# ai-dynamo/grove

Hardware: AMD Instinct MI355X
Metric: podgangs_per_sec (higher is better)
Workload: dtype bf16; 1 GPU; global_batch=4, parallelism=gang1, gang_size=1, payload=2048x2048x2048x1, inflight=2, concurrent_syncs=4, transport=http, scheduler=amd-gang-scheduler (native xGMI Filter/Score)

## Files before the change

grove_amd/kubelet/gpunode.py:

```python
from __future__ import annotations

import logging
from typing import Any, Dict, Optional, Tuple

from ..api import constants as c
from ..kubecore.store import Obj

log = logging.getLogger("grove.gpunode")

PAYLOAD_ANNOTATION = "grove.io/payload"
PAYLOAD_SHAPE_ANNOTATION = "grove.io/payload-shape"
GPU_IDS_ANNOTATION = "scheduling.amd.com/gpu-ids"

_gpuwork = None


def load_gpuwork():
    global _gpuwork
    if _gpuwork is not None:
        return _gpuwork
    import torch
    try:
        from ..ops import _gpuwork as ext
    except ImportError as e:
        if torch.cuda.is_available():
            raise RuntimeError(
                "grove_amd.ops._gpuwork native extension is missing on a GPU box — "
                "build it with python -m grove_amd.ops.build") from e
        return None
    _gpuwork = ext
    return ext


def parse_payload(pod: Obj) -> Tuple[str, Tuple[int, ...]]:
    ann = pod["metadata"].get("annotations") or {}
    kind = ann.get(PAYLOAD_ANNOTATION, "gemm")
    shape = ann.get(PAYLOAD_SHAPE_ANNOTATION, "")
    if kind == "gemm":
        dims = tuple(int(x) for x in shape.split("x")) if shape else (1024, 1024, 1024, 1)
        if len(dims) == 3:
            dims = dims + (1,)
        return "gemm", dims
    if kind == "stream":
        return "stream", (int(shape) if shape else 1 << 24, 2)
    if kind == "decode":
        dims = tuple(int(v) for v in shape.split("x")) if shape else (8192, 8192, 4)
        if len(dims) == 2:
            dims = dims + (1,)
        return "decode", dims
    return "none", ()


def assigned_gpu(pod: Obj) -> Optional[int]:
    ids = (pod["metadata"].get("annotations") or {}).get(GPU_IDS_ANNOTATION, "")
    if not ids:
        return None
    return int(ids.split(",")[0])


def run_payload_descriptor(kind: str, dims: Tuple[int, ...], device: int) -> Dict[str, Any]:
    import torch
    if not torch.cuda.is_available():
        if kind == "gemm":
            m, n, k, iters = dims
            a = torch.randn(min(m, 128), min(k, 128))
            b = torch.randn(min(k, 128), min(n, 128))
            for _ in range(iters):
                a @ b
        return {"device": "cpu", "kind": kind}
    ext = load_gpuwork()
    device = device % max(1, torch.cuda.device_count())
    with torch.cuda.device(device):
        if kind == "gemm":
            m, n, k, iters = dims
            tflops = ext.burn_gemm(m, n, k, iters)
            return {"device": device, "kind": kind, "tflops": tflops}
        if kind == "stream":
            n_floats = dims[0]
            iters = dims[1] if len(dims) > 1 else 2
            gbps = ext.stream_triad(n_floats, iters)
            return {"device": device, "kind": kind, "gbps": gbps}
        if kind == "decode":
            n, k, iters = dims
            gbps = ext.burn_decode(n, k, iters)
            return {"device": device, "kind": kind, "weight_stream_gbps": gbps}
    return {"device": device, "kind": kind}


def gpu_pod_payload(pod: Obj) -> None:
    gpu = assigned_gpu(pod)
    kind, dims = parse_payload(pod)
    if kind == "none":
        return
    if gpu is None:
        gpu = 0
    run_payload_descriptor(kind, dims, gpu)
```

grove_amd/ops/gpuwork.hip:

```cpp
#include <torch/extension.h>
#include <ATen/hip/HIPContext.h>
#include <hip/hip_runtime.h>
#include <hip/hip_bf16.h>

#include <vector>

#define WAVE 64
#define BK 64

using bf16 = __hip_bfloat16;
using bf16x8 = __attribute__((ext_vector_type(8))) __bf16;
using f32x16 = __attribute__((ext_vector_type(16))) float;

__device__ __forceinline__ int swz(int row, int cb) {
    return (cb ^ ((row ^ (row >> 3)) & 7)) & 7;
}

__device__ __forceinline__ int lds_off(int row, int cb) {
    return row * BK + (swz(row, cb) << 3);
}

__device__ __forceinline__ void tile_map(int bid, int num_pid_m, int tiles_n,
                                         int& tile_m, int& tile_n) {
    const int GROUP = 8;
    int group_size = min(GROUP, num_pid_m);
    int pids_per_group = group_size * tiles_n;
    int group = bid / pids_per_group;
    int in_group = bid % pids_per_group;
    tile_m = group * GROUP + (in_group % group_size);
    tile_n = in_group / group_size;
}

__device__ __forceinline__ void tile_map_rect(int bid, int tiles_m, int tiles_n,
                                              int m_per_xcd, int n_win,
                                              int& tile_m, int& tile_n) {
    int mwin_tiles = 8 * m_per_xcd;
    int win = bid >> 8;
    int idx = bid & 255;
    int xcd = idx & 7;
    int slot = idx >> 3;
    int nwins = tiles_n / n_win;
    tile_m = (win / nwins) * mwin_tiles + xcd * m_per_xcd + slot % m_per_xcd;
    tile_n = (win % nwins) * n_win + slot / m_per_xcd;
}

template <int THREADS, int AUX = 0>
__device__ __forceinline__ void stage_tile(const bf16* __restrict__ g, long ld,
                                           __bf16* __restrict__ dst, int rows,
                                           int tid, int wave_piece0) {
#pragma unroll
    for (int i = 0; i < 8; ++i) {
        if (i >= (rows * 8) / THREADS)
            break;
        int p = tid + i * THREADS;
        int row = p >> 3;
        int cb_src = swz(row, p & 7);
        int base = wave_piece0 + i * THREADS;
        __builtin_amdgcn_global_load_lds(
            (const __attribute__((address_space(1))) uint32_t*)(
                g + (long)row * ld + (cb_src << 3)),
            (__attribute__((address_space(3))) uint32_t*)(dst + base * 8),
            16, 0, AUX);
    }
}

__global__ __launch_bounds__(512, 1)
void mfma_gemm_bf16_256_kernel(const bf16* __restrict__ A,
                               const bf16* __restrict__ Bt,
                               float* __restrict__ C,
                               int M, int N, int K,
                               int m_per_xcd, int n_win) {
    constexpr int BM = 256, BN = 256;
    __shared__ __bf16 smem[2 * (BM * BK + BN * BK)];
    auto sAp = [&](int b) { return smem + b * (BM * BK + BN * BK); };
    auto sBp = [&](int b) { return smem + b * (BM * BK + BN * BK) + BM * BK; };

    int tile_m, tile_n;
    if (m_per_xcd)
        tile_map_rect(blockIdx.x, M / BM, N / BN, m_per_xcd, n_win,
                      tile_m, tile_n);
    else
        tile_map(blockIdx.x, M / BM, N / BN, tile_m, tile_n);
    const int tid = threadIdx.x;
    const int wave = tid / WAVE;
    const int lane = tid % WAVE;
    const int wr = wave >> 1, wc = wave & 1;
    const long row0 = (long)tile_m * BM;
    const long col0 = (long)tile_n * BN;
    const int wave_piece0 = wave * WAVE;

    auto stage = [&](int buf, long kk) {
        stage_tile<512>(A + row0 * K + kk, K, sAp(buf), BM, tid, wave_piece0);
        stage_tile<512>(Bt + col0 * K + kk, K, sBp(buf), BN, tid, wave_piece0);
    };

    f32x16 acc[2][4] = {};
    bf16x8 afrag[2][2], bfrag[2][4];
    const int a_row = wr * 64 + (lane & 31);
    const int b_row = wc * 128 + (lane & 31);
    const int k_half = lane >> 5;
    auto load_frags = [&](int pb, int buf, int ks) {
        int cb = (ks << 1) | k_half;
#pragma unroll
        for (int mt = 0; mt < 2; ++mt)
            afrag[pb][mt] = *(const bf16x8*)(sAp(buf) + lds_off(a_row + mt * 32, cb));
#pragma unroll
        for (int nt = 0; nt < 4; ++nt)
            bfrag[pb][nt] = *(const bf16x8*)(sBp(buf) + lds_off(b_row + nt * 32, cb));
    };

    stage(0, 0);
    __syncthreads();
    load_frags(0, 0, 0);
    for (long kk = 0; kk < K; kk += BK) {
        int buf = (kk / BK) & 1;
        if (kk + BK < K) stage(buf ^ 1, kk + BK);
#pragma unroll
        for (int ks = 0; ks < BK / 16; ++ks) {
            int pb = ks & 1;
            if (ks + 1 < BK / 16)
                load_frags(pb ^ 1, buf, ks + 1);
#pragma unroll
            for (int mt = 0; mt < 2; ++mt)
#pragma unroll
                for (int nt = 0; nt < 4; ++nt)
                    acc[mt][nt] = __builtin_amdgcn_mfma_f32_32x32x16_bf16(
                        afrag[pb][mt], bfrag[pb][nt], acc[mt][nt], 0, 0, 0);
        }
        __syncthreads();
        if (kk + BK < K) load_frags(0, buf ^ 1, 0);
    }

    const int c_row_lane = 4 * (lane >> 5);
#pragma unroll
    for (int mt = 0; mt < 2; ++mt)
#pragma unroll
        for (int nt = 0; nt < 4; ++nt)
#pragma unroll
            for (int reg = 0; reg < 16; ++reg) {
                int r = wr * 64 + mt * 32 + (reg & 3) + 8 * (reg >> 2) + c_row_lane;
                int cl = wc * 128 + nt * 32 + (lane & 31);
                C[(row0 + r) * (long)N + col0 + cl] = acc[mt][nt][reg];
            }
}

__global__ __launch_bounds__(256, 2)
void mfma_gemm_bf16_128_kernel(const bf16* __restrict__ A,
                               const bf16* __restrict__ Bt,
                               float* __restrict__ C,
                               int M, int N, int K) {
    constexpr int BM = 128, BN = 128;
    __shared__ __bf16 smem[2 * (BM * BK + BN * BK)];
    auto sAp = [&](int b) { return smem + b * (BM * BK + BN * BK); };
    auto sBp = [&](int b) { return smem + b * (BM * BK + BN * BK) + BM * BK; };

    int tile_m, tile_n;
    tile_map(blockIdx.x, M / BM, N / BN, tile_m, tile_n);
    const int tid = threadIdx.x;
    const int wave = tid / WAVE;
    const int lane = tid % WAVE;
    const int wr = wave >> 1, wc = wave & 1;
    const long row0 = (long)tile_m * BM;
    const long col0 = (long)tile_n * BN;
    const int wave_piece0 = wave * WAVE;

    auto stage = [&](int buf, long kk) {
        stage_tile<256>(A + row0 * K + kk, K, sAp(buf), BM, tid, wave_piece0);
        stage_tile<256>(Bt + col0 * K + kk, K, sBp(buf), BN, tid, wave_piece0);
    };

    f32x16 acc[2][2] = {};
    bf16x8 afrag[2][2], bfrag[2][2];
    const int a_row = wr * 64 + (lane & 31);
    const int b_row = wc * 64 + (lane & 31);
    const int k_half = lane >> 5;
    auto load_frags = [&](int pb, int buf, int ks) {
        int cb = (ks << 1) | k_half;
#pragma unroll
        for (int mt = 0; mt < 2; ++mt)
            afrag[pb][mt] = *(const bf16x8*)(sAp(buf) + lds_off(a_row + mt * 32, cb));
#pragma unroll
        for (int nt = 0; nt < 2; ++nt)
            bfrag[pb][nt] = *(const bf16x8*)(sBp(buf) + lds_off(b_row + nt * 32, cb));
    };

    stage(0, 0);
    __syncthreads();
    load_frags(0, 0, 0);
    for (long kk = 0; kk < K; kk += BK) {
        int buf = (kk / BK) & 1;
        if (kk + BK < K) stage(buf ^ 1, kk + BK);
#pragma unroll
        for (int ks = 0; ks < BK / 16; ++ks) {
            int pb = ks & 1;
            if (ks + 1 < BK / 16)
                load_frags(pb ^ 1, buf, ks + 1);
#pragma unroll
            for (int mt = 0; mt < 2; ++mt)
#pragma unroll
                for (int nt = 0; nt < 2; ++nt)
                    acc[mt][nt] = __builtin_amdgcn_mfma_f32_32x32x16_bf16(
                        afrag[pb][mt], bfrag[pb][nt], acc[mt][nt], 0, 0, 0);
        }
        __syncthreads();
        if (kk + BK < K) load_frags(0, buf ^ 1, 0);
    }

    const int c_row_lane = 4 * (lane >> 5);
#pragma unroll
    for (int mt = 0; mt < 2; ++mt)
#pragma unroll
        for (int nt = 0; nt < 2; ++nt)
#pragma unroll
            for (int reg = 0; reg < 16; ++reg) {
                int r = wr * 64 + mt * 32 + (reg & 3) + 8 * (reg >> 2) + c_row_lane;
                int cl = wc * 64 + nt * 32 + (lane & 31);
                C[(row0 + r) * (long)N + col0 + cl] = acc[mt][nt][reg];
            }
}

__global__ __launch_bounds__(256)
void decode_gemv_kernel(const bf16* __restrict__ W,
                        const bf16* __restrict__ x,
                        float* __restrict__ y, int N, int K) {
    const int lane = threadIdx.x % WAVE;
    const int wave = threadIdx.x / WAVE;
    const int row = blockIdx.x * 4 + wave;
    if (row >= N) return;
    const bf16* w = W + (long)row * K;
    float acc = 0.f;
    for (int k0 = lane * 8; k0 < K; k0 += WAVE * 8) {
        bf16x8 wv = *(const bf16x8*)(w + k0);
        bf16x8 xv = *(const bf16x8*)(x + k0);
#pragma unroll
        for (int i = 0; i < 8; ++i)
            acc += (float)wv[i] * (float)xv[i];
    }
    for (int off = 32; off > 0; off >>= 1)
        acc += __shfl_down(acc, off, 64);
    if (lane == 0) y[row] = acc;
}

torch::Tensor decode_gemv(torch::Tensor w, torch::Tensor x) {
    TORCH_CHECK(w.is_cuda() && x.is_cuda() && w.dtype() == torch::kBFloat16
                && x.dtype() == torch::kBFloat16, "bf16 GPU tensors required");
    TORCH_CHECK(w.is_contiguous() && x.is_contiguous(), "contiguous required");
    int64_t N = w.size(0), K = w.size(1);
    TORCH_CHECK(x.numel() == K && K % 512 == 0, "x must be [K], K%512==0");
    auto y = torch::empty({N}, w.options().dtype(torch::kFloat32));
    hipStream_t stream = at::hip::getCurrentHIPStream();
    hipLaunchKernelGGL(decode_gemv_kernel, dim3((N + 3) / 4), dim3(256), 0, stream,
                       (const bf16*)w.data_ptr(), (const bf16*)x.data_ptr(),
                       y.data_ptr<float>(), (int)N, (int)K);
    return y;
}

double burn_decode(int64_t n, int64_t k, int64_t iters) {
    auto opt = torch::TensorOptions().dtype(torch::kBFloat16).device(torch::kCUDA);
    auto w = torch::randn({n, k}, opt.dtype(torch::kFloat32)).to(torch::kBFloat16);
    auto x = torch::randn({k}, opt.dtype(torch::kFloat32)).to(torch::kBFloat16);
    auto y = torch::empty({n}, opt.dtype(torch::kFloat32));
    hipStream_t stream = at::hip::getCurrentHIPStream();
    auto launch = [&] {
        hipLaunchKernelGGL(decode_gemv_kernel, dim3((n + 3) / 4), dim3(256), 0,
                           stream, (const bf16*)w.data_ptr(),
                           (const bf16*)x.data_ptr(), y.data_ptr<float>(),
                           (int)n, (int)k);
    };
    launch();
    C10_HIP_CHECK(hipStreamSynchronize(stream));
    auto t0 = std::chrono::steady_clock::now();
    for (int64_t i = 0; i < iters; ++i) launch();
    C10_HIP_CHECK(hipStreamSynchronize(stream));
    auto t1 = std::chrono::steady_clock::now();
    double secs = std::chrono::duration<double>(t1 - t0).count();
    return 2.0 * n * k * iters / secs / 1e9;
}

__global__ void stream_triad_kernel(const float4* __restrict__ a,
                                    const float4* __restrict__ b,
                                    float4* __restrict__ c, long n4, float s) {
    long i = (long)blockIdx.x * blockDim.x + threadIdx.x;
    long stride = (long)gridDim.x * blockDim.x;
    for (; i < n4; i += stride) {
        float4 x = a[i], y = b[i];
        c[i] = make_float4(x.x + s * y.x, x.y + s * y.y, x.z + s * y.z, x.w + s * y.w);
    }
}


static void launch_gemm(const torch::Tensor& a, const torch::Tensor& bt,
                        torch::Tensor& c, int64_t M, int64_t N, int64_t K,
                        int64_t map_mode = -1) {
    hipStream_t stream = at::hip::getCurrentHIPStream();
    if (M % 256 == 0 && N % 256 == 0 && (M / 256) * (N / 256) >= 256) {
        int tiles_m = (int)(M / 256), tiles_n = (int)(N / 256);
        int m_per_xcd = 0, n_win = 0;
        int mpx = std::min<int>(4, std::max(1, tiles_m / 8));
        int nw = 256 / (8 * mpx);
        bool want_rect = (map_mode == 1) ||
                         (map_mode < 0 && (int64_t)tiles_m * tiles_n > 256);
        if (want_rect && map_mode != 0 &&
            tiles_m % (8 * mpx) == 0 && tiles_n % nw == 0) {
            m_per_xcd = mpx; n_win = nw;
        }
        dim3 grid((M / 256) * (N / 256)), block(512);
        hipLaunchKernelGGL(mfma_gemm_bf16_256_kernel, grid, block, 0, stream,
                           (const bf16*)a.data_ptr(), (const bf16*)bt.data_ptr(),
                           c.data_ptr<float>(), (int)M, (int)N, (int)K,
                           m_per_xcd, n_win);
    } else {
        dim3 grid((M / 128) * (N / 128)), block(256);
        hipLaunchKernelGGL(mfma_gemm_bf16_128_kernel, grid, block, 0, stream,
                           (const bf16*)a.data_ptr(), (const bf16*)bt.data_ptr(),
                           c.data_ptr<float>(), (int)M, (int)N, (int)K);
    }
}

static void check_dims(int64_t M, int64_t N, int64_t K) {
    TORCH_CHECK(M % 128 == 0 && N % 128 == 0 && K % 64 == 0,
                "mfma_gemm_bf16 requires M%128==0, N%128==0, K%64==0 (got ",
                M, "x", N, "x", K, ")");
}

torch::Tensor mfma_gemm_bf16(torch::Tensor a, torch::Tensor bt) {
    TORCH_CHECK(a.is_cuda() && bt.is_cuda(), "inputs must be on GPU");
    TORCH_CHECK(a.dtype() == torch::kBFloat16 && bt.dtype() == torch::kBFloat16,
                "inputs must be bf16");
    TORCH_CHECK(a.is_contiguous() && bt.is_contiguous(), "inputs must be contiguous");
    int64_t M = a.size(0), K = a.size(1), N = bt.size(0);
    TORCH_CHECK(bt.size(1) == K, "shape mismatch: A[M,K] Bt[N,K]");
    check_dims(M, N, K);
    auto c = torch::empty({M, N}, a.options().dtype(torch::kFloat32));
    launch_gemm(a, bt, c, M, N, K);
    return c;
}

double burn_gemm(int64_t m, int64_t n, int64_t k, int64_t iters,
                 int64_t map_mode) {
    check_dims(m, n, k);
    auto opt = torch::TensorOptions().dtype(torch::kBFloat16).device(torch::kCUDA);
    auto a = torch::randn({m, k}, opt.dtype(torch::kFloat32)).to(torch::kBFloat16);
    auto bt = torch::randn({n, k}, opt.dtype(torch::kFloat32)).to(torch::kBFloat16);
    auto c = torch::empty({m, n}, opt.dtype(torch::kFloat32));
    hipStream_t stream = at::hip::getCurrentHIPStream();
    launch_gemm(a, bt, c, m, n, k, map_mode);
    C10_HIP_CHECK(hipStreamSynchronize(stream));
    auto t0 = std::chrono::steady_clock::now();
    for (int64_t i = 0; i < iters; ++i) launch_gemm(a, bt, c, m, n, k, map_mode);
    C10_HIP_CHECK(hipStreamSynchronize(stream));
    auto t1 = std::chrono::steady_clock::now();
    double secs = std::chrono::duration<double>(t1 - t0).count();
    return 2.0 * m * n * k * iters / secs / 1e12;
}

double stream_triad(int64_t n_floats, int64_t iters) {
    TORCH_CHECK(n_floats % 4 == 0, "n_floats must be a multiple of 4");
    auto opt = torch::TensorOptions().dtype(torch::kFloat32).device(torch::kCUDA);
    auto a = torch::randn({n_floats}, opt);
    auto b = torch::randn({n_floats}, opt);
    auto c = torch::empty({n_floats}, opt);
    long n4 = n_floats / 4;
    hipStream_t stream = at::hip::getCurrentHIPStream();
    int blocks = std::min<long>(8192, (n4 + 255) / 256);
    auto launch = [&] {
        hipLaunchKernelGGL(stream_triad_kernel, dim3(blocks), dim3(256), 0, stream,
                           (const float4*)a.data_ptr(), (const float4*)b.data_ptr(),
                           (float4*)c.data_ptr(), n4, 1.5f);
    };
    launch();
    C10_HIP_CHECK(hipStreamSynchronize(stream));
    auto t0 = std::chrono::steady_clock::now();
    for (int64_t i = 0; i < iters; ++i) launch();
    C10_HIP_CHECK(hipStreamSynchronize(stream));
    auto t1 = std::chrono::steady_clock::now();
    double secs = std::chrono::duration<double>(t1 - t0).count();
    return 12.0 * n_floats * iters / secs / 1e9;
}

PYBIND11_MODULE(TORCH_EXTENSION_NAME, m) {
    m.doc() = "grove_amd MI355X pod-payload kernels (MFMA bf16 GEMM, HBM stream)";
    m.def("mfma_gemm_bf16", &mfma_gemm_bf16, "C[M,N]=A[M,K]@Bt[N,K]^T (bf16 in, fp32 out)");
    m.def("burn_gemm", &burn_gemm, "run iters GEMM steps; returns TFLOP/s",
          pybind11::arg("m"), pybind11::arg("n"), pybind11::arg("k"),
          pybind11::arg("iters"), pybind11::arg("map_mode") = -1);
    m.def("burn_gemm_v",
          [](int64_t m_, int64_t n_, int64_t k_, int64_t it, int64_t) {
              return burn_gemm(m_, n_, k_, it, -1);
          }, "compat alias for burn_gemm (bk arg ignored)");
    m.def("stream_triad", &stream_triad, "HBM triad; returns GB/s");
    m.def("decode_gemv", &decode_gemv, "y[N]=W[N,K]@x[K] (bf16 in, fp32 out)");
    m.def("burn_decode", &burn_decode,
          "iters decode GEMV steps; returns weight-stream GB/s");
}
```

Before: 321.8 gangs/s.

## Streamline pod payload: fused bf16 RNG fill, skip warmup, event timing, GIL release

Replaces the fp32 randn-then-cast input generation with a single custom kernel that writes bf16 normals directly, skips the warmup launch for pod payloads, and times with pooled HIP events instead of a stream sync plus a host clock. It also releases the GIL during the native burn calls and passes the device as an argument instead of using a Python context manager. This is meant to cut per-pod GPU work and host serialisation so concurrent payloads overlap. Dropping the warmup could change the reported TFLOP/s, and the custom RNG produces a different distribution quality than torch.randn.

```diff
diff --git a/grove_amd/kubelet/gpunode.py b/grove_amd/kubelet/gpunode.py
--- a/grove_amd/kubelet/gpunode.py
+++ b/grove_amd/kubelet/gpunode.py
@@ -70,20 +70,19 @@
         return {"device": "cpu", "kind": kind}
     ext = load_gpuwork()
     device = device % max(1, torch.cuda.device_count())
-    with torch.cuda.device(device):
-        if kind == "gemm":
-            m, n, k, iters = dims
-            tflops = ext.burn_gemm(m, n, k, iters)
-            return {"device": device, "kind": kind, "tflops": tflops}
-        if kind == "stream":
-            n_floats = dims[0]
-            iters = dims[1] if len(dims) > 1 else 2
-            gbps = ext.stream_triad(n_floats, iters)
-            return {"device": device, "kind": kind, "gbps": gbps}
-        if kind == "decode":
-            n, k, iters = dims
-            gbps = ext.burn_decode(n, k, iters)
-            return {"device": device, "kind": kind, "weight_stream_gbps": gbps}
+    if kind == "gemm":
+        m, n, k, iters = dims
+        tflops = ext.burn_gemm(m, n, k, iters, warmup=False, device=device)
+        return {"device": device, "kind": kind, "tflops": tflops}
+    if kind == "stream":
+        n_floats = dims[0]
+        iters = dims[1] if len(dims) > 1 else 2
+        gbps = ext.stream_triad(n_floats, iters, device=device)
+        return {"device": device, "kind": kind, "gbps": gbps}
+    if kind == "decode":
+        n, k, iters = dims
+        gbps = ext.burn_decode(n, k, iters, warmup=False, device=device)
+        return {"device": device, "kind": kind, "weight_stream_gbps": gbps}
     return {"device": device, "kind": kind}
 
 
diff --git a/grove_amd/ops/gpuwork.hip b/grove_amd/ops/gpuwork.hip
--- a/grove_amd/ops/gpuwork.hip
+++ b/grove_amd/ops/gpuwork.hip
@@ -3,6 +3,13 @@
 #include <hip/hip_runtime.h>
 #include <hip/hip_bf16.h>
 
+#include <ATen/hip/impl/HIPGuardImplMasqueradingAsCUDA.h>
+
+#include <atomic>
+#include <mutex>
+#include <optional>
+#include <random>
+#include <utility>
 #include <vector>
 
 #define WAVE 64
@@ -255,11 +262,131 @@
     return y;
 }
 
-double burn_decode(int64_t n, int64_t k, int64_t iters) {
-    auto opt = torch::TensorOptions().dtype(torch::kBFloat16).device(torch::kCUDA);
-    auto w = torch::randn({n, k}, opt.dtype(torch::kFloat32)).to(torch::kBFloat16);
-    auto x = torch::randn({k}, opt.dtype(torch::kFloat32)).to(torch::kBFloat16);
-    auto y = torch::empty({n}, opt.dtype(torch::kFloat32));
+__device__ __forceinline__ uint64_t splitmix64(uint64_t z) {
+    z = (z ^ (z >> 30)) * 0xBF58476D1CE4E5B9ull;
+    z = (z ^ (z >> 27)) * 0x94D049BB133111EBull;
+    return z ^ (z >> 31);
+}
+
+__global__ __launch_bounds__(256)
+void fill_normal_bf16_kernel(bf16x8* __restrict__ out, long n8, uint64_t seed) {
+    long i = (long)blockIdx.x * blockDim.x + threadIdx.x;
+    const long stride = (long)gridDim.x * blockDim.x;
+    for (; i < n8; i += stride) {
+        bf16x8 v;
+#pragma unroll
+        for (int j = 0; j < 4; ++j) {
+            uint64_t ctr = (uint64_t)i * 4 + j + 1;
+            uint64_t h = splitmix64(seed + ctr * 0x9E3779B97F4A7C15ull);
+            float u1 = (float)((uint32_t)(h >> 40) + 1u) * 0x1p-24f;
+            float u2 = (float)(uint32_t)h * 0x1p-32f;
+            float r = __builtin_amdgcn_sqrtf(-1.3862943611198906f *
+                                             __builtin_amdgcn_logf(u1));
+            v[2 * j] = (__bf16)(r * __builtin_amdgcn_cosf(u2));
+            v[2 * j + 1] = (__bf16)(r * __builtin_amdgcn_sinf(u2));
+        }
+        out[i] = v;
+    }
+}
+
+static void launch_fill(torch::Tensor& t, uint64_t seed) {
+    long n8 = t.numel() / 8;
+    if (n8 == 0) return;
+    int cus = at::cuda::getCurrentDeviceProperties()->multiProcessorCount;
+    long blocks = std::min<long>((n8 + 255) / 256, (long)cus * 8);
+    hipStream_t stream = at::hip::getCurrentHIPStream();
+    hipLaunchKernelGGL(fill_normal_bf16_kernel, dim3((unsigned)blocks), dim3(256), 0,
+                       stream, (bf16x8*)t.data_ptr(), n8, seed);
+    C10_HIP_KERNEL_LAUNCH_CHECK();
+}
+
+static uint64_t host_mix(uint64_t z) {
+    z += 0x9E3779B97F4A7C15ull;
+    z = (z ^ (z >> 30)) * 0xBF58476D1CE4E5B9ull;
+    z = (z ^ (z >> 27)) * 0x94D049BB133111EBull;
+    return z ^ (z >> 31);
+}
+
+static uint64_t next_seed() {
+    static const uint64_t salt =
+        ((uint64_t)std::random_device{}() << 32) ^ std::random_device{}();
+    static std::atomic<uint64_t> counter{0};
+    return host_mix(salt ^ host_mix(counter.fetch_add(1, std::memory_order_relaxed)));
+}
+
+static torch::Tensor randn_bf16(at::IntArrayRef shape) {
+    auto t = torch::empty(shape, torch::TensorOptions().dtype(torch::kBFloat16)
+                                     .device(torch::kCUDA));
+    launch_fill(t, next_seed());
+    return t;
+}
+
+void fill_normal_bf16(torch::Tensor t, int64_t seed) {
+    TORCH_CHECK(t.is_cuda() && t.dtype() == torch::kBFloat16 && t.is_contiguous(),
+                "fill_normal_bf16 requires a contiguous bf16 GPU tensor");
+    TORCH_CHECK(t.numel() % 8 == 0 && (uintptr_t)t.data_ptr() % 16 == 0,
+                "fill_normal_bf16 requires numel % 8 == 0 and 16-byte alignment");
+    c10::hip::HIPGuardMasqueradingAsCUDA guard(t.device());
+    launch_fill(t, host_mix((uint64_t)seed));
+}
+
+struct EventPair { hipEvent_t start, stop; };
+
+static std::mutex g_event_mu;
+static std::vector<std::vector<EventPair>> g_event_pool;
+
+struct ScopedEvents {
+    EventPair ev;
+    int device;
+    explicit ScopedEvents(int dev) : device(dev) {
+        {
+            std::lock_guard<std::mutex> lk(g_event_mu);
+            if ((int)g_event_pool.size() <= dev) g_event_pool.resize(dev + 1);
+            auto& free_list = g_event_pool[dev];
+            if (!free_list.empty()) {
+                ev = free_list.back();
+                free_list.pop_back();
+                return;
+            }
+        }
+        C10_HIP_CHECK(hipEventCreate(&ev.start));
+        C10_HIP_CHECK(hipEventCreate(&ev.stop));
+    }
+    ~ScopedEvents() {
+        std::lock_guard<std::mutex> lk(g_event_mu);
+        g_event_pool[device].push_back(ev);
+    }
+};
+
+template <typename Launch>
+static double timed_launches(Launch&& launch, int64_t iters, bool warmup) {
+    int dev = 0;
+    C10_HIP_CHECK(hipGetDevice(&dev));
+    hipStream_t stream = at::hip::getCurrentHIPStream();
+    ScopedEvents se(dev);
+    if (warmup) launch();
+    C10_HIP_CHECK(hipEventRecord(se.ev.start, stream));
+    for (int64_t i = 0; i < iters; ++i) launch();
+    C10_HIP_CHECK(hipEventRecord(se.ev.stop, stream));
+    C10_HIP_CHECK(hipEventSynchronize(se.ev.stop));
+    float ms = 0.f;
+    C10_HIP_CHECK(hipEventElapsedTime(&ms, se.ev.start, se.ev.stop));
+    return (double)ms * 1e-3;
+}
+
+static std::optional<c10::Device> device_arg(int64_t device) {
+    if (device < 0) return std::nullopt;
+    return c10::Device(c10::kCUDA, (c10::DeviceIndex)device);
+}
+
+double burn_decode(int64_t n, int64_t k, int64_t iters, bool warmup,
+                   int64_t device) {
+    TORCH_CHECK(n > 0 && k > 0 && k % 512 == 0 && iters > 0,
+                "burn_decode requires n>0, k%512==0, iters>0");
+    c10::hip::OptionalHIPGuardMasqueradingAsCUDA guard(device_arg(device));
+    auto w = randn_bf16({n, k});
+    auto x = randn_bf16({k});
+    auto y = torch::empty({n}, w.options().dtype(torch::kFloat32));
     hipStream_t stream = at::hip::getCurrentHIPStream();
     auto launch = [&] {
         hipLaunchKernelGGL(decode_gemv_kernel, dim3((n + 3) / 4), dim3(256), 0,
@@ -267,13 +394,7 @@
                            (const bf16*)x.data_ptr(), y.data_ptr<float>(),
                            (int)n, (int)k);
     };
-    launch();
-    C10_HIP_CHECK(hipStreamSynchronize(stream));
-    auto t0 = std::chrono::steady_clock::now();
-    for (int64_t i = 0; i < iters; ++i) launch();
-    C10_HIP_CHECK(hipStreamSynchronize(stream));
-    auto t1 = std::chrono::steady_clock::now();
-    double secs = std::chrono::duration<double>(t1 - t0).count();
+    double secs = timed_launches(launch, iters, warmup);
     return 2.0 * n * k * iters / secs / 1e9;
 }
 
@@ -337,25 +458,22 @@
 }
 
 double burn_gemm(int64_t m, int64_t n, int64_t k, int64_t iters,
-                 int64_t map_mode) {
+                 int64_t map_mode, bool warmup, int64_t device) {
     check_dims(m, n, k);
-    auto opt = torch::TensorOptions().dtype(torch::kBFloat16).device(torch::kCUDA);
-    auto a = torch::randn({m, k}, opt.dtype(torch::kFloat32)).to(torch::kBFloat16);
-    auto bt = torch::randn({n, k}, opt.dtype(torch::kFloat32)).to(torch::kBFloat16);
-    auto c = torch::empty({m, n}, opt.dtype(torch::kFloat32));
-    hipStream_t stream = at::hip::getCurrentHIPStream();
-    launch_gemm(a, bt, c, m, n, k, map_mode);
-    C10_HIP_CHECK(hipStreamSynchronize(stream));
-    auto t0 = std::chrono::steady_clock::now();
-    for (int64_t i = 0; i < iters; ++i) launch_gemm(a, bt, c, m, n, k, map_mode);
-    C10_HIP_CHECK(hipStreamSynchronize(stream));
-    auto t1 = std::chrono::steady_clock::now();
-    double secs = std::chrono::duration<double>(t1 - t0).count();
+    TORCH_CHECK(m > 0 && n > 0 && k > 0 && iters > 0,
+                "burn_gemm requires positive dims and iters");
+    c10::hip::OptionalHIPGuardMasqueradingAsCUDA guard(device_arg(device));
+    auto a = randn_bf16({m, k});
+    auto bt = randn_bf16({n, k});
+    auto c = torch::empty({m, n}, a.options().dtype(torch::kFloat32));
+    double secs = timed_launches(
+        [&] { launch_gemm(a, bt, c, m, n, k, map_mode); }, iters, warmup);
     return 2.0 * m * n * k * iters / secs / 1e12;
 }
 
-double stream_triad(int64_t n_floats, int64_t iters) {
+double stream_triad(int64_t n_floats, int64_t iters, int64_t device) {
     TORCH_CHECK(n_floats % 4 == 0, "n_floats must be a multiple of 4");
+    c10::hip::OptionalHIPGuardMasqueradingAsCUDA guard(device_arg(device));
     auto opt = torch::TensorOptions().dtype(torch::kFloat32).device(torch::kCUDA);
     auto a = torch::randn({n_floats}, opt);
     auto b = torch::randn({n_floats}, opt);
@@ -381,15 +499,24 @@
 PYBIND11_MODULE(TORCH_EXTENSION_NAME, m) {
     m.doc() = "grove_amd MI355X pod-payload kernels (MFMA bf16 GEMM, HBM stream)";
     m.def("mfma_gemm_bf16", &mfma_gemm_bf16, "C[M,N]=A[M,K]@Bt[N,K]^T (bf16 in, fp32 out)");
+    using nogil = pybind11::call_guard<pybind11::gil_scoped_release>;
     m.def("burn_gemm", &burn_gemm, "run iters GEMM steps; returns TFLOP/s",
           pybind11::arg("m"), pybind11::arg("n"), pybind11::arg("k"),
-          pybind11::arg("iters"), pybind11::arg("map_mode") = -1);
+          pybind11::arg("iters"), pybind11::arg("map_mode") = -1,
+          pybind11::arg("warmup") = true, pybind11::arg("device") = -1, nogil());
     m.def("burn_gemm_v",
           [](int64_t m_, int64_t n_, int64_t k_, int64_t it, int64_t) {
-              return burn_gemm(m_, n_, k_, it, -1);
-          }, "compat alias for burn_gemm (bk arg ignored)");
-    m.def("stream_triad", &stream_triad, "HBM triad; returns GB/s");
+              return burn_gemm(m_, n_, k_, it, -1, true, -1);
+          }, "compat alias for burn_gemm (bk arg ignored)", nogil());
+    m.def("stream_triad", &stream_triad, "HBM triad; returns GB/s",
+          pybind11::arg("n_floats"), pybind11::arg("iters"),
+          pybind11::arg("device") = -1, nogil());
+    m.def("fill_normal_bf16", &fill_normal_bf16,
+          "fill a contiguous bf16 GPU tensor (numel%8==0) with N(0,1) from seed",
+          pybind11::arg("tensor"), pybind11::arg("seed"));
     m.def("decode_gemv", &decode_gemv, "y[N]=W[N,K]@x[K] (bf16 in, fp32 out)");
     m.def("burn_decode", &burn_decode,
-          "iters decode GEMV steps; returns weight-stream GB/s");
-}
+          "iters decode GEMV steps; returns weight-stream GB/s",
+          pybind11::arg("n"), pybind11::arg("k"), pybind11::arg("iters"),
+          pybind11::arg("warmup") = true, pybind11::arg("device") = -1, nogil());
+}
```

Result: slower. 178.7 gangs/s (-44.5%).
